# kimkyeonghun/MSA

Hardware: AMD Instinct MI355X
Metric: train-step samples/sec (higher is better)
Workload: dtype bf16

## Files before the change

msa_amd/csrc/rowwise.hip:

```cpp
#include "common.h"
#include <cstring>

std::atomic<int> g_mmb_deterministic{0};

__global__ void split_rows_kernel(const int64_t* __restrict__ row_seq, const int64_t* __restrict__ row_pos, const int* __restrict__ start_a,
                                  const int* __restrict__ start_b, const int* __restrict__ valid, int mode, int M, int rows_a,
                                  int64_t* __restrict__ perm, int64_t* __restrict__ inv, const int* __restrict__ rank,
                                  int* __restrict__ perm32, int* __restrict__ inv32) {
    const int i = blockIdx.x * blockDim.x + threadIdx.x;
    if (i >= M) return;
    const int s = (int)row_seq[i], p = rank ? rank[i] : (int)row_pos[i], v = valid[s];
    int n = rows_a;
    bool own = false;
    if (p < v) { n = start_a[s] + p; own = true; }
    else if (mode == 0) { n = start_b[s] + p - v; own = true; }
    else if (mode == 1) { n = start_b[s]; own = p == v; }
    inv[i] = n;
    if (inv32) inv32[i] = n;
    if (own) { perm[n] = i; if (perm32) perm32[n] = i; }
}

#define SL_MAXSEQ 1024
__global__ __launch_bounds__(1024) void split_layout_kernel(const int* __restrict__ lens, const int* __restrict__ valid, int nseq, int rows, int xs,
                                                            int nf_max, int nq_max, int* __restrict__ out) {
// ... 452 lines not shown
        if (r.dyr >= 0) {
            const bf16_t* dyr = dy + (size_t)r.dyr * lddy + lane * 4;
#pragma unroll
            for (int c = 0; c < NV; ++c) ndl[c] = *(const u32x2_t*)(dyr + c * 256);
        } else {
#pragma unroll
            for (int c = 0; c < NV; ++c) ndl[c] = (u32x2_t){0u, 0u};
        }
    };
    int i = blockIdx.x * WPB + w;
    if (i < M) {
        Row r0 = row_of(i);
        request(r0);
        Row r1 = row_of(i + stride);
        for (; i < M; i += stride) {
            u32x2_t dl[NV], tl[NV];
#pragma unroll
            for (int c = 0; c < NV; ++c) { dl[c] = ndl[c]; tl[c] = ntl[c]; }
            const Row r = r0;
            r0 = r1;
            if (i + stride < M) request(r0);
            r1 = row_of(i + 2 * stride);
            const uint32_t row_w = r.dr * (uint32_t)((H / 2) * MMB_WEYL);
            const float nmr = -r.mean * r.rstd;
            f32x2 g[NV][2], xh[NV][2], s1 = {0.f, 0.f}, s2 = {0.f, 0.f};
#pragma unroll
            for (int c = 0; c < NV; ++c)
#pragma unroll
                for (int k = 0; k < 2; ++k) {
                    uint32_t dw = dl[c][k];
                    if (POST) dw &= ~mmb_drop_mask2(mmb_pair_mix(row_w + lane_post + (uint32_t)(c * 128 + k) * MMB_WEYL), post_pk);
                    f32x2 dv = bf2_unpack(dw);
                    if (POST) dv *= post_scale;
                    xh[c][k] = fma2(bf2_unpack(tl[c][k]), (f32x2){r.rstd, r.rstd}, (f32x2){nmr, nmr});
                    ag[c][k] = fma2(dv, xh[c][k], ag[c][k]);
                    ab[c][k] += dv;
                    g[c][k] = dv * gam[c][k];
                    s1 += g[c][k];
                    s2 = fma2(g[c][k], xh[c][k], s2);
                }
            const float m1 = wave_sum_dpp(s1.x + s1.y) * (1.0f / H), m2 = wave_sum_dpp(s2.x + s2.y) * (1.0f / H);
            const float c1 = -m1 * r.rstd, c2 = -m2 * r.rstd;
            bf16_t* dxr = dx + (size_t)r.dxr * lddx + lane * 4;
            bf16_t* dx2r = DX2 ? dx2 + (size_t)i * lddx2 + lane * 4 : nullptr;
#pragma unroll
            for (int c = 0; c < NV; ++c) {
                u32x2_t ow, ow2;
#pragma unroll
                for (int k = 0; k < 2; ++k) {
                    const f32x2 o = fma2(xh[c][k], (f32x2){c2, c2}, fma2(g[c][k], (f32x2){r.rstd, r.rstd}, (f32x2){c1, c1}));
                    ow[k] = bf2_pack(o);
                    if (DX2 && PRE) {
                        const f32x2 o2 = o * pre_scale;
                        const uint32_t dm = mmb_drop_mask2(mmb_pair_mix(row_w + lane_pre + (uint32_t)(c * 128 + k) * MMB_WEYL), pre_pk);
                        ow2[k] = bf2_pack(o2) & ~dm;
                        const float klo = (dm & 0x8000u) ? 0.f : o2[0], khi = (dm & 0x80000000u) ? 0.f : o2[1];
                        ad[c][k] += (f32x2){klo, khi};
                    } else {
                        if (DX2) ow2[k] = ow[k];
                        if (want_ad) ad[c][k] += o;
                    }
                }
                *(u32x2_t*)(dxr + c * 256) = ow;
                if (DX2) *(u32x2_t*)(dx2r + c * 256) = ow2;
            }
        }
    }
    auto fold = [&](f32x2 (&acc)[NV][2], int slot, float* out) {
#pragma unroll
        for (int c = 0; c < NV; ++c)
#pragma unroll
            for (int k = 0; k < 2; ++k) *(f32x2*)&red[w][c * 256 + lane * 4 + 2 * k] = acc[c][k];
        __syncthreads();
        for (int col = threadIdx.x; col < H; col += WPB * 64) {
            float t = 0.f;
#pragma unroll
            for (int q = 0; q < WPB; ++q) t += red[q][col];
            if (partial) partial[((size_t)blockIdx.x * 3 + slot) * H + col] = t;
            else if (out) atomicAdd(out + col, t);
        }
        __syncthreads();
    };
    fold(ag, 0, dgamma);
    fold(ab, 1, dbeta);
    if (dbias2) fold(ad, 2, dbias2);
}


struct LnReduceBatch { float* out[32][3]; const float* partial[32]; int nblocks[32]; int H, nq, items, ordered; };
__global__ __launch_bounds__(1024) void ln_bwd_reduce_batch_kernel(const LnReduceBatch b) {
    __shared__ float red[16][64];
    const int col = blockIdx.x * 64 + (threadIdx.x & 63), sub = threadIdx.x >> 6, nsub = (int)blockDim.x >> 6;
    const int item = blockIdx.y / b.nq, k = blockIdx.y - item * b.nq;
    float* out = b.out[item][k];
    if (out == nullptr) return;
    if (b.ordered) {
        for (int j = 0; j < item; ++j)
            if (b.out[j][k] == out) return;
        float total = 0.f;
        for (int it = item; it < b.items; ++it) {
            if (b.out[it][k] != out) continue;
            const float* partial = b.partial[it];
            const int nblocks = b.nblocks[it];
            float s = 0.f;
            if (col < b.H)
                for (int q = sub; q < nblocks; q += nsub) s += partial[((size_t)q * b.nq + k) * b.H + col];
            red[sub][threadIdx.x & 63] = s;
            __syncthreads();
            if (sub == 0) {
                float t = red[0][threadIdx.x];
                for (int q = 1; q < nsub; ++q) t += red[q][threadIdx.x];
                total += t;
            }
            __syncthreads();
        }
        if (sub == 0 && col < b.H) out[col] += total;
        return;
    }
    const float* partial = b.partial[item];
    const int nblocks = b.nblocks[item];
    const int per = (nblocks + gridDim.z - 1) / gridDim.z;
    const int b0 = blockIdx.z * per, b1 = min(nblocks, b0 + per);
    float s = 0.f;
    if (col < b.H)
        for (int q = b0 + sub; q < b1; q += nsub) s += partial[((size_t)q * b.nq + k) * b.H + col];
    red[sub][threadIdx.x & 63] = s;
    __syncthreads();
    if (sub == 0 && col < b.H) {
        float t = red[0][threadIdx.x];
        for (int q = 1; q < nsub; ++q) t += red[q][threadIdx.x];
        atomicAdd(out + col, t);
    }
}

__global__ __launch_bounds__(256) void embed_gather_kernel(const int64_t* __restrict__ ids, const int64_t* __restrict__ tts,
                                                           const float* __restrict__ word, const float* __restrict__ type,
                                                           const float* __restrict__ pos, int n, int T, int H, int V,
                                                           bf16_t* __restrict__ out, int ldo) {
    const int lane = threadIdx.x & 63;
    for (int i = blockIdx.x * 4 + (threadIdx.x >> 6); i < n; i += gridDim.x * 4) {
        long id = ids[i]; if (id < 0 || id >= V) id = 0;
        const long tt = tts ? (tts[i] != 0) : 0;
        const float* wr = word + (size_t)id * H;
        const float* tr = type + (size_t)tt * H;
        const float* pr = pos + (size_t)(i % T) * H;
        for (int col = lane * 4; col < H; col += 256) {
            const float4 a = *(const float4*)(wr + col), b = *(const float4*)(tr + col), c = *(const float4*)(pr + col);
            bf16x4 o = {f2bf(a.x + b.x + c.x), f2bf(a.y + b.y + c.y), f2bf(a.z + b.z + c.z), f2bf(a.w + b.w + c.w)};
            *(bf16x4*)(out + (size_t)i * ldo + col) = o;
        }
    }
}

__global__ __launch_bounds__(256) void embed_scatter_kernel(const int64_t* __restrict__ ids, const int64_t* __restrict__ tts,
                                                            const bf16_t* __restrict__ d, int ldd, int n, int T, int H, int V,
                                                            float* __restrict__ gword, float* __restrict__ gtype, float* __restrict__ gpos,
                                                            float* __restrict__ type_slab) {
    const int p = blockIdx.x;
    for (int col = threadIdx.x * 4; col < H; col += 1024) {
        float ps[4] = {0.f, 0.f, 0.f, 0.f}, t0[4] = {0.f, 0.f, 0.f, 0.f}, t1[4] = {0.f, 0.f, 0.f, 0.f};
        for (int i0 = p + (int)blockIdx.y * 8 * T; i0 < n; i0 += 8 * T * (int)gridDim.y) {
            long id[8]; bool tt[8]; bf16x4 v[8];
#pragma unroll
            for (int u = 0; u < 8; ++u) {
                const int i = min(i0 + u * T, n - 1);
                id[u] = ids[i];
                tt[u] = tts ? (tts[i] != 0) : false;
                v[u] = *(const bf16x4*)(d + (size_t)i * ldd + col);
            }
#pragma unroll
            for (int u = 0; u < 8; ++u) {
                if (i0 + u * T >= n) break;
                const bool word = gword != nullptr && id[u] > 0 && id[u] < V;
#pragma unroll
                for (int r = 0; r < 4; ++r) {
                    const float f = bf2f(v[u][r]);
                    ps[r] += f;
                    if (tt[u]) t1[r] += f; else t0[r] += f;
                    if (word) atomicAdd(gword + (size_t)id[u] * H + col + r, f);
                }
            }
        }
#pragma unroll
        for (int r = 0; r < 4; ++r) {
            atomicAdd(gpos + (size_t)p * H + col + r, ps[r]);
            if (type_slab) { type_slab[((size_t)p * 2) * H + col + r] = t0[r]; type_slab[((size_t)p * 2 + 1) * H + col + r] = t1[r]; }
            else {
                if (t0[r] != 0.f) atomicAdd(gtype + col + r, t0[r]);
                if (t1[r] != 0.f) atomicAdd(gtype + H + col + r, t1[r]);
            }
        }
    }
}

template <int KSHIFT, typename FT>
__global__ __launch_bounds__(256) void pair_proj_fwd_kernel(const FT* __restrict__ feat, int n_rows, int P, int D,
                                                            const float* __restrict__ W, const float* __restrict__ bias, int H,
                                                            bf16_t* __restrict__ out, int ldo, int T, int KC, int pitch) {
#if defined(__gfx950__)
    extern __shared__ __attribute__((aligned(16))) float pair_sm[];
    float* Ws = pair_sm;
    float* Fs = pair_sm + 128 * pitch;
    const int tid = threadIdx.x, wave = tid >> 6, lane = tid & 63, c = lane & 15, g = lane >> 4;
    const int row0 = blockIdx.x * 64, h0 = blockIdx.y * 128;
    const int wh = (wave & 1) * 64, wr = (wave >> 1) * 32;
    f32x4 acc[4][2];
#pragma unroll
    for (int i = 0; i < 4; ++i)
#pragma unroll
        for (int j = 0; j < 2; ++j) acc[i][j] = (f32x4){0.f, 0.f, 0.f, 0.f};
    float bcol[4][4];
#pragma unroll
    for (int i = 0; i < 4; ++i)
#pragma unroll
        for (int q = 0; q < 4; ++q) bcol[i][q] = bias[min(h0 + wh + 16 * i + 4 * g + q, H - 1)];
    constexpr int kw = 1 << KSHIFT, rstep = 256 >> KSHIFT;
    const int kl = tid & (kw - 1), rsub = tid >> KSHIFT;
    for (int k0 = 0; k0 < D; k0 += KC) {
        const int kc = min(KC, D - k0), kc4 = (kc + 3) & ~3;
        if (k0) __syncthreads();
        const float kmask = kl < kc ? 1.f : 0.f;
        const int kg = min(k0 + kl, D - 1);
        const bool kst = kl < kc4;
        auto stage = [&](auto base, int g0, int lim, int lrow0, auto nrows_c) {
            constexpr int N = decltype(nrows_c)::value / rstep, NB = N < 32 ? N : 32;
#pragma unroll 1
            for (int ub = 0; ub < N; ub += NB) {
                std::remove_cv_t<std::remove_reference_t<decltype(base[0])>> v[NB];
#pragma unroll
                for (int u = 0; u < NB; ++u) {
                    const int gr = g0 + rsub + (ub + u) * rstep;
                    v[u] = base[(uint32_t)(min(gr, lim - 1) * D + kg)];
                }
                if (kst) {
#pragma unroll
                    for (int u = 0; u < NB; ++u) {
                        const int r = rsub + (ub + u) * rstep;
                        pair_sm[(lrow0 + r) * pitch + kl] = (float)v[u] * (g0 + r < lim ? kmask : 0.f);
                    }
                }
            }
        };
        stage(W, h0, H, 0, std::integral_constant<int, 128>{});
        stage(feat, row0, n_rows, 128, std::integral_constant<int, 64>{});
        __syncthreads();
        const float* wa = Ws + (wh + c) * pitch + g;
        const float* fb = Fs + (wr + c) * pitch + g;
        float av[4], bv[2];
#pragma unroll
        for (int i = 0; i < 4; ++i) av[i] = wa[16 * i * pitch];
#pragma unroll
        for (int j = 0; j < 2; ++j) bv[j] = fb[16 * j * pitch];
        for (int kk = 0; kk < kc4; kk += 4) {
            float an[4], bn[2];
            const int kn = kk + 4 < kc4 ? kk + 4 : kk;
#pragma unroll
            for (int i = 0; i < 4; ++i) an[i] = wa[16 * i * pitch + kn];
#pragma unroll
            for (int j = 0; j < 2; ++j) bn[j] = fb[16 * j * pitch + kn];
            __builtin_amdgcn_sched_barrier(0);
#pragma unroll
            for (int i = 0; i < 4; ++i)
#pragma unroll
                for (int j = 0; j < 2; ++j) acc[i][j] = __builtin_amdgcn_mfma_f32_16x16x4f32(av[i], bv[j], acc[i][j], 0, 0, 0);
            __builtin_amdgcn_sched_barrier(0);
#pragma unroll
            for (int i = 0; i < 4; ++i) av[i] = an[i];
#pragma unroll
            for (int j = 0; j < 2; ++j) bv[j] = bn[j];
        }
    }
    if (h0 + 128 <= H && !(ldo & 7)) {
        __syncthreads();
        bf16_t* Os = (bf16_t*)pair_sm;
#pragma unroll
        for (int j = 0; j < 2; ++j)
#pragma unroll
            for (int i = 0; i < 4; ++i) {
                bf16x4 ov = {f2bf(fmaxf(acc[i][j][0] + bcol[i][0], 0.f)), f2bf(fmaxf(acc[i][j][1] + bcol[i][1], 0.f)),
                             f2bf(fmaxf(acc[i][j][2] + bcol[i][2], 0.f)), f2bf(fmaxf(acc[i][j][3] + bcol[i][3], 0.f))};
                *(bf16x4*)(Os + (wr + 16 * j + c) * 136 + wh + 16 * i + 4 * g) = ov;
            }
        __syncthreads();
#pragma unroll
        for (int ps = 0; ps < 4; ++ps) {
            const int rl = (tid >> 4) + 16 * ps, row = row0 + rl;
            if (row >= n_rows) continue;
            const int b_ = row / P, p_ = row - b_ * P;
            *(bf16x8*)(out + (size_t)(b_ * (T + P) + T + p_) * ldo + h0 + 8 * (tid & 15)) = *(const bf16x8*)(Os + rl * 136 + 8 * (tid & 15));
        }
        return;
    }
#pragma unroll
    for (int j = 0; j < 2; ++j) {
        const int row = row0 + wr + 16 * j + c;
        if (row >= n_rows) continue;
        const int b_ = row / P, p_ = row - b_ * P;
        bf16_t* orow = out + (size_t)(b_ * (T + P) + T + p_) * ldo;
#pragma unroll
        for (int i = 0; i < 4; ++i) {
            const int h = h0 + wh + 16 * i + 4 * g;
            if (h + 3 < H && !(ldo & 3)) {
                bf16x4 ov = {f2bf(fmaxf(acc[i][j][0] + bcol[i][0], 0.f)), f2bf(fmaxf(acc[i][j][1] + bcol[i][1], 0.f)),
                             f2bf(fmaxf(acc[i][j][2] + bcol[i][2], 0.f)), f2bf(fmaxf(acc[i][j][3] + bcol[i][3], 0.f))};
                *(bf16x4*)(orow + h) = ov;
            } else {
#pragma unroll
                for (int q = 0; q < 4; ++q) if (h + q < H) orow[h + q] = f2bf(fmaxf(acc[i][j][q] + bcol[i][q], 0.f));
            }
        }
    }
#endif
}

struct PairBwdArgs { const void* feat; const bf16_t* J; const bf16_t* dJ; float* slab; int n, P, D, T, H, ld, rows_per_wg, ntiles; };
constexpr int PAIR_NT = 5;

template <typename FT>
__global__ __launch_bounds__(256) void pair_wgrad_kernel(const PairBwdArgs a) {
#if defined(__gfx950__)
    __shared__ float red[3][PAIR_NT * 16][64];
    const int tid = threadIdx.x, wave = tid >> 6, lane = tid & 63, c = lane & 15, g = lane >> 4;
    const int hb = blockIdx.x * 64, s = blockIdx.y, jt0 = blockIdx.z * PAIR_NT;
    const int njt = min(PAIR_NT, a.ntiles - jt0);
    const int rpw = a.rows_per_wg >> 2;
    const int r0 = s * a.rows_per_wg + wave * rpw, r1 = min(r0 + rpw, a.n);
    const int hcol = hb + 4 * c;
    const bool hok = hcol + 3 < a.H;
    struct Stage { bf16x4 j, d; float f[PAIR_NT]; };
    auto load = [&](Stage& st, int r) {
        const bool ok = r < r1;
        const int rc = ok ? r : 0;
        const int b_ = rc / a.P, p_ = rc - b_ * a.P;
        const size_t off = (size_t)(b_ * (a.T + a.P) + a.T + p_) * a.ld + (hok ? hcol : 0);
        st.j = *(const bf16x4*)(a.J + off);
        st.d = *(const bf16x4*)(a.dJ + off);
        const FT* fr = (const FT*)a.feat + (size_t)rc * a.D;
#pragma unroll
        for (int j = 0; j < PAIR_NT; ++j) {
            const int k = (jt0 + j) * 16 + c;
            const float live = (ok && j < njt) ? 1.0f : 0.0f;
            st.f[j] = fmaf((float)fr[min(k, a.D - 1)], k < a.D ? live : 0.0f, k == a.D ? live : 0.0f);
        }
// ... 12 lines not shown
#pragma unroll
        for (int u = 0; u < 4; ++u) {
            float av[4];
#pragma unroll
            for (int i = 0; i < 4; ++i) av[i] = bf2f(st[u].j[i]) > 0.f ? bf2f(st[u].d[i]) : 0.f;
            float fv[PAIR_NT];
#pragma unroll
            for (int j = 0; j < PAIR_NT; ++j) fv[j] = st[u].f[j];
            load(st[u], r + 16 + 4 * u + g);
#pragma unroll
            for (int j = 0; j < PAIR_NT; ++j) {
                if (j >= njt) continue;
#pragma unroll
                for (int i = 0; i < 4; ++i) acc[j][i] = __builtin_amdgcn_mfma_f32_16x16x4f32(av[i], fv[j], acc[j][i], 0, 0, 0);
            }
        }
    }
    if (wave) {
#pragma unroll
        for (int j = 0; j < PAIR_NT; ++j)
#pragma unroll
            for (int i = 0; i < 4; ++i)
#pragma unroll
                for (int q = 0; q < 4; ++q) red[wave - 1][(j * 4 + i) * 4 + q][lane] = acc[j][i][q];
    }
    __syncthreads();
    if (wave == 0) {
        const int W1 = a.D + 1;
        float* out = a.slab + (size_t)s * a.H * W1;
#pragma unroll
        for (int j = 0; j < PAIR_NT; ++j) {
            const int k = (jt0 + j) * 16 + c;
#pragma unroll
            for (int i = 0; i < 4; ++i)
#pragma unroll
                for (int q = 0; q < 4; ++q) {
                    const int e = (j * 4 + i) * 4 + q;
                    const float v = ((acc[j][i][q] + red[0][e][lane]) + red[1][e][lane]) + red[2][e][lane];
                    const int h = hb + 4 * (4 * g + q) + i;
                    if (j < njt && k < W1 && h < a.H) out[(size_t)h * W1 + k] = v;
                }
        }
    }
#endif
}

__global__ void pair_wgrad_reduce_kernel(const float* __restrict__ slab, int S, int H, int D, float* __restrict__ dW, float* __restrict__ db) {
    const int i = blockIdx.x * blockDim.x + threadIdx.x;
    const int W1 = D + 1;
    if (i >= H * W1) return;
    float t = 0.f;
    int s_ = 0;
    for (; s_ + 8 <= S; s_ += 8) {
        float v[8];
#pragma unroll
        for (int u = 0; u < 8; ++u) v[u] = slab[(size_t)(s_ + u) * H * W1 + i];
#pragma unroll
        for (int u = 0; u < 8; ++u) t += v[u];
    }
    for (; s_ < S; ++s_) t += slab[(size_t)s_ * H * W1 + i];
    const int h = i / W1, k = i - h * W1;
    if (k < D) dW[(size_t)h * D + k] += t; else db[h] += t;
}

__global__ __launch_bounds__(1024) void active_rows_kernel(const int64_t* __restrict__ labels, int M, int V, int* __restrict__ idx, int* __restrict__ count) {
    __shared__ int wsum[16];
    __shared__ int base;
    const int tid = threadIdx.x, lane = tid & 63, w = tid >> 6;
    if (tid == 0) base = 0;
    __syncthreads();
    for (int i0 = 0; i0 < M; i0 += 1024) {
        const int i = i0 + tid;
        const bool act = i < M && labels[i] >= 0 && labels[i] < V;
        const unsigned long long bal = __ballot(act);
        const int before = __popcll(bal & ((1ull << lane) - 1ull));
        if (lane == 0) wsum[w] = __popcll(bal);
        __syncthreads();
        int off = base;
        for (int q = 0; q < w; ++q) off += wsum[q];
        if (act) idx[off + before] = i;
        __syncthreads();
        if (tid == 0) { int t = 0; for (int q = 0; q < 16; ++q) t += wsum[q]; base += t; }
        __syncthreads();
    }
    if (tid == 0) *count = base;
}

__global__ void ce_count_kernel(const int64_t* __restrict__ labels, int M, int V, const int* __restrict__ seg_bounds, int nseg,
                                float* __restrict__ inv_count, float* __restrict__ loss_sum) {
    __shared__ int cnt[4];
    if (threadIdx.x < 4) cnt[threadIdx.x] = 0;
    __syncthreads();
    const int b1 = nseg > 1 ? seg_bounds[1] : 0x7fffffff, b2 = nseg > 2 ? seg_bounds[2] : 0x7fffffff, b3 = nseg > 3 ? seg_bounds[3] : 0x7fffffff;
    int c[4] = {0, 0, 0, 0};
    for (int i0 = threadIdx.x; i0 < M; i0 += (int)blockDim.x * 8) {
        int64_t lab[8];
#pragma unroll
        for (int u = 0; u < 8; ++u) lab[u] = labels[min(i0 + u * (int)blockDim.x, M - 1)];
#pragma unroll
        for (int u = 0; u < 8; ++u) {
            const int i = i0 + u * (int)blockDim.x;
            const int ok = (i < M && lab[u] >= 0 && lab[u] < V) ? 1 : 0;
            const int sg = (i >= b1 ? 1 : 0) + (i >= b2 ? 1 : 0) + (i >= b3 ? 1 : 0);
#pragma unroll
            for (int q = 0; q < 4; ++q) c[q] += (sg == q) ? ok : 0;
        }
    }
#pragma unroll
    for (int q = 0; q < 4; ++q) if (c[q]) atomicAdd(&cnt[q], c[q]);
    __syncthreads();
    if (threadIdx.x < nseg) {
        inv_count[threadIdx.x] = 1.0f / (float)max(cnt[threadIdx.x], 1);
        loss_sum[threadIdx.x] = 0.f;
    }
}

__global__ __launch_bounds__(1024) void ce_loss_sum_ordered_kernel(const float* __restrict__ row_loss, int M, const int* __restrict__ seg_bounds, int nseg,
                                                                   float* __restrict__ loss_sum) {
    __shared__ float red[4][1024];
    const int b1 = nseg > 1 ? seg_bounds[1] : 0x7fffffff, b2 = nseg > 2 ? seg_bounds[2] : 0x7fffffff, b3 = nseg > 3 ? seg_bounds[3] : 0x7fffffff;
    float c[4] = {0.f, 0.f, 0.f, 0.f};
    for (int i0 = threadIdx.x; i0 < M; i0 += 1024 * 8) {
        float v[8];
#pragma unroll
        for (int u = 0; u < 8; ++u) v[u] = row_loss[min(i0 + u * 1024, M - 1)];
#pragma unroll
        for (int u = 0; u < 8; ++u) {
            const int i = i0 + u * 1024;
            const int sg = (i >= b1 ? 1 : 0) + (i >= b2 ? 1 : 0) + (i >= b3 ? 1 : 0);
            const float x = i < M ? v[u] : 0.f;
#pragma unroll
            for (int q = 0; q < 4; ++q) c[q] += (sg == q) ? x : 0.f;
        }
    }
#pragma unroll
    for (int q = 0; q < 4; ++q) red[q][threadIdx.x] = c[q];
    __syncthreads();
    for (int w = 512; w > 0; w >>= 1) {
        if ((int)threadIdx.x < w) {
#pragma unroll
            for (int q = 0; q < 4; ++q) red[q][threadIdx.x] += red[q][threadIdx.x + w];
        }
        __syncthreads();
    }
    if ((int)threadIdx.x < nseg) loss_sum[threadIdx.x] = red[threadIdx.x][0];
}

#define RUNS_MAXN 8192
__global__ __launch_bounds__(1024) void id_runs_sum_rows_kernel(const void* __restrict__ src, int src_bf16, int lds, const int64_t* __restrict__ ids,
                                                                int n, int H, int V, const int64_t* __restrict__ uni, int U,
                                                                float* __restrict__ dst, int ldd) {
    __shared__ int list[RUNS_MAXN];
    __shared__ float red[1024 * 4];
    __shared__ int s_count, s_earlier;
    const int i0 = blockIdx.x, tid = threadIdx.x, nthr = blockDim.x;
    const long long key = ids[i0];
    if (key <= 0 || key >= V) return;
    if (tid == 0) { s_count = 0; s_earlier = 0; }
    __syncthreads();
    int earlier = 0;
    for (int j = tid; j < i0; j += nthr) earlier |= (ids[j] == key) ? 1 : 0;
    if (earlier) s_earlier = 1;
    __syncthreads();
    if (s_earlier) return;
    long long dr = key;
    if (uni) {
        int lo = 0, hi = U - 1;
        while (lo < hi) { const int mid = (lo + hi) >> 1; if (uni[mid] < key) lo = mid + 1; else hi = mid; }
        if (U <= 0 || uni[lo] != key) return;
        dr = lo;
    }
    if (tid < 64) {
        int count = 0;
        for (int base = i0; base < n; base += 64) {
            const int j = base + tid;
            const bool hit = j < n && ids[j] == key;
            const unsigned long long m = __ballot(hit);
            if (hit) list[count + __popcll(m & ((1ull << tid) - 1ull))] = j;
            count += __popcll(m);
        }
        if (tid == 0) s_count = count;
    }
    __syncthreads();
    const int cnt = s_count;
    const int CT = H >> 2, G = nthr / CT;
    const int g = tid / CT, c = tid - g * CT;
    float a[4] = {0.f, 0.f, 0.f, 0.f};
    if (g < G) {
#pragma unroll 4
        for (int k = g; k < cnt; k += G) {
            const size_t r = (size_t)list[k];
            if (src_bf16) {
                const bf16x4 x = *(const bf16x4*)((const bf16_t*)src + r * lds + 4 * c);
#pragma unroll
                for (int q = 0; q < 4; ++q) a[q] += bf2f(x[q]);
            } else {
                const float4 x = *(const float4*)((const float*)src + r * lds + 4 * c);
                a[0] += x.x; a[1] += x.y; a[2] += x.z; a[3] += x.w;
            }
        }
#pragma unroll
        for (int q = 0; q < 4; ++q) red[(g * CT + c) * 4 + q] = a[q];
    }
    __syncthreads();
    if (g == 0) {
        float4* d = (float4*)(dst + (size_t)dr * ldd + 4 * c);
        float4 o = *d;
        float t[4] = {0.f, 0.f, 0.f, 0.f};
        for (int gg = 0; gg < G; ++gg)
#pragma unroll
            for (int q = 0; q < 4; ++q) t[q] += red[(gg * CT + c) * 4 + q];
        o.x += t[0]; o.y += t[1]; o.z += t[2]; o.w += t[3];
        *d = o;
    }
}

__global__ void embed_type_fold_kernel(const float* __restrict__ slab, int T, int H, float* __restrict__ gtype) {
    const int e = blockIdx.x * blockDim.x + threadIdx.x;
    if (e >= 2 * H) return;
    float t = 0.f;
    for (int p = 0; p < T; ++p) t += slab[(size_t)p * 2 * H + e];
    gtype[e] += t;
}

#define CE_MAXC 16
template <int MODE, bool F32, bool SMOOTH = false>
__global__ __launch_bounds__(256) void ce_row_kernel(const void* __restrict__ logits_, int ldv, int V, const int64_t* __restrict__ labels,
                                                     const int* __restrict__ seg_bounds, int nseg, const float* __restrict__ inv_count,
                                                     float* __restrict__ loss_sum, float* __restrict__ row_lse, const float* __restrict__ gscale,
                                                     bf16_t* __restrict__ dlogits, int ldd, const int* __restrict__ rows, float* __restrict__ row_loss,
                                                     float one_minus, float eps_over_v) {
    __shared__ float red[4];
    __shared__ float lab_logit;
    const int i = rows ? rows[blockIdx.x] : blockIdx.x;
    const int64_t lab = labels[i];
    const int tid = threadIdx.x, lane = tid & 63, w = tid >> 6;
    const int nchunk = ldv >> 3;
    if (lab < 0 || lab >= V) {
        if (MODE == 0) { if (tid == 0) { row_lse[i] = 0.f; if (row_loss) row_loss[i] = 0.f; } }
        else {
            bf16_t* drow = dlogits + (size_t)(rows ? blockIdx.x : i) * ldd;
            const bf16x8 z = {0, 0, 0, 0, 0, 0, 0, 0};
            for (int c = tid; c < nchunk; c += 256) *(bf16x8*)(drow + c * 8) = z;
        }
        return;
    }
    int s = 0;
    while (s + 1 < nseg && i >= seg_bounds[s + 1]) ++s;
    bf16x8 v[CE_MAXC];
    if constexpr (F32) {
        const float* row = (const float*)logits_ + (size_t)i * ldv;
#pragma unroll
        for (int c = 0; c < CE_MAXC; ++c) {
            const int ch = c * 256 + tid;
            if (ch < nchunk) {
                const float4 lo = *(const float4*)(row + ch * 8), hi = *(const float4*)(row + ch * 8 + 4);
                v[c] = (bf16x8){f2bf(lo.x), f2bf(lo.y), f2bf(lo.z), f2bf(lo.w), f2bf(hi.x), f2bf(hi.y), f2bf(hi.z), f2bf(hi.w)};
            }
        }
    } else {
        const bf16_t* row = (const bf16_t*)logits_ + (size_t)i * ldv;
#pragma unroll
        for (int c = 0; c < CE_MAXC; ++c) {
            const int ch = c * 256 + tid;
            if (ch < nchunk) v[c] = *(const bf16x8*)(row + ch * 8);
        }
    }
    if (MODE == 0) {
        float mx = -INFINITY;
#pragma unroll
        for (int c = 0; c < CE_MAXC; ++c) {
            const int ch = c * 256 + tid;
            if (ch < nchunk) {
#pragma unroll
                for (int r = 0; r < 8; ++r) if (ch * 8 + r < V) mx = fmaxf(mx, bf2f(v[c][r]));
            }
        }
        mx = wave_max(mx);
        if (lane == 0) red[w] = mx;
        __syncthreads();
        mx = fmaxf(fmaxf(red[0], red[1]), fmaxf(red[2], red[3]));
        __syncthreads();
        float se = 0.f;
        float sx = 0.f;
#pragma unroll
        for (int c = 0; c < CE_MAXC; ++c) {
            const int ch = c * 256 + tid;
            if (ch < nchunk) {
#pragma unroll
                for (int r = 0; r < 8; ++r) if (ch * 8 + r < V) {
                    se += __expf(bf2f(v[c][r]) - mx);
                    if constexpr (SMOOTH) sx += bf2f(v[c][r]);
                }
                if ((int)(lab >> 3) == ch) lab_logit = bf2f(v[c][lab & 7]);
            }
        }
        se = wave_sum(se);
        if (lane == 0) red[w] = se;
        if constexpr (SMOOTH) {
            __shared__ float red_x[4];
            sx = wave_sum(sx);
            if (lane == 0) red_x[w] = sx;
            __syncthreads();
            if (tid == 0) {
                const float lse = mx + __logf(red[0] + red[1] + red[2] + red[3]);
                const float sum_x = ((red_x[0] + red_x[1]) + red_x[2]) + red_x[3];
                row_lse[i] = lse;
                const float term = __fmaf_rn(-eps_over_v, sum_x, __fmaf_rn(-one_minus, lab_logit, lse)) * inv_count[s];
                if (row_loss) row_loss[i] = term;
                else atomicAdd(loss_sum + s, term);
            }
            return;
        }
        __syncthreads();
        if (tid == 0) {
            const float lse = mx + __logf(red[0] + red[1] + red[2] + red[3]);
            row_lse[i] = lse;
            if (row_loss) row_loss[i] = (lse - lab_logit) * inv_count[s];
            else atomicAdd(loss_sum + s, (lse - lab_logit) * inv_count[s]);
        }
    } else {
        const float lse = row_lse[i];
        const float scale = inv_count[s] * gscale[s];
        bf16_t* drow = dlogits + (size_t)(rows ? blockIdx.x : i) * ldd;
#pragma unroll
        for (int c = 0; c < CE_MAXC; ++c) {
            const int ch = c * 256 + tid;
            if (ch < nchunk) {
                bf16x8 o;
#pragma unroll
                for (int r = 0; r < 8; ++r) {
                    const int col = ch * 8 + r;
                    float pr = col < V ? __expf(bf2f(v[c][r]) - lse) : 0.f;
                    if constexpr (SMOOTH) {
                        if (col == (int)lab) pr -= one_minus;
                        if (col < V) pr -= eps_over_v;
                    } else {
                        if (col == (int)lab) pr -= 1.0f;
                    }
                    o[r] = f2bf(pr * scale);
                }
                *(bf16x8*)(drow + ch * 8) = o;
            }
        }
    }
}

typedef uint32_t vt_u32x4 __attribute__((ext_vector_type(4)));

__device__ __forceinline__ uint32_t vt_key(uint32_t h) {
    const uint32_t neg = (uint32_t)((int32_t)h >> 31);
    return h ^ ((neg & 0x7FFF0000u) | 0x80000000u);
}
__device__ __forceinline__ float vt_value(uint32_t word) {
    const uint32_t kk = word & 0xFFFF0000u;
    return __builtin_bit_cast(float, (kk & 0x80000000u) ? (kk ^ 0x80000000u) : (kk ^ 0xFFFF0000u));
}
__device__ __forceinline__ uint32_t vt_wave_max(uint32_t v) {
#pragma unroll
    for (int o = 32; o > 0; o >>= 1) v = max(v, (uint32_t)__shfl_xor((int)v, o, 64));
    return v;
}
template <bool COUNT>
__device__ __forceinline__ uint32_t vt_scan(const uint32_t (&e)[CE_MAXC * 8], uint32_t prev, uint32_t lab_word, int& above) {
    uint32_t best = 0u;
#pragma unroll
    for (int n = 0; n < CE_MAXC * 8; ++n) {
        best = max(best, e[n] - prev);
        if (COUNT) above += e[n] > lab_word ? 1 : 0;
    }
    const uint32_t word = best + prev;
    return word < prev ? word : 0u;
}

// ... 745 lines not shown
        if (int e = mmb_allow_lds((const void*)pair_proj_fwd_kernel<7, FT>, 192 * 130 * (int)sizeof(float), attr_done)) return e;
        hipLaunchKernelGGL((pair_proj_fwd_kernel<7, FT>), dim3((n + 63) / 64, (H + 127) / 128), dim3(256), lds, stream, feat, n, P, D, W, bias, H, (bf16_t*)out, ldo, T,
                           KC, pitch);
    }
    MMB_CHECK_LAUNCH();
    return 0;
}

extern "C" {

uint32_t mmbert_rng_stream(uint64_t seed, uint32_t site) {
    uint32_t a = mmb_hash32((uint32_t)seed ^ 0xA511E9B3u);
    uint32_t b = mmb_hash32((uint32_t)(seed >> 32) + 0x7F4A7C15u);
    return mmb_hash32(a ^ (b * 0x9E3779B1u) ^ mmb_hash32(site * 0x85EBCA6Bu + 0x27D4EB2Fu));
}

uint32_t mmbert_dropout_thr16(float p) {
    if (p <= 0.f) return 0;
    double t = (double)p * 65536.0 + 0.5;
    if (t > 65535.0) t = 65535.0;
    return (uint32_t)t;
}

static inline bool ln_lean(int H) { return (H & 255) == 0 && H <= LN_MAXV * 256; }

int mmbert_ln_fwd(hipStream_t stream, const void* x, int ldx, const int* in_rows, void* y, int ldy, const int* out_rows,
                  int M, int H, const float* gamma, const float* beta, float eps, float* mean, float* rstd,
                  uint32_t dstream, uint32_t dthr, float dscale, int drop_row0) {
    if (M <= 0) return 0;
    if (H > LN_MAXV * 256 || (H & 3) || (ldx & 3) || (ldy & 3)) return -1;
    constexpr int cap = 0;
    if (ln_lean(H)) {
        const int NVL = H >> 8;
        const dim3 grid(grid_for(M, 4, cap > 0 ? cap : 1024));
#define LN_FWD_LEAN(NVV, DD) hipLaunchKernelGGL((ln_fwd_lean_kernel<NVV, DD>), grid, dim3(256), 0, stream, (const bf16_t*)x, ldx, in_rows, \
                                                 (bf16_t*)y, ldy, out_rows, M, gamma, beta, eps, mean, rstd, dstream, dthr, dscale, drop_row0)
        if (dthr) { if (NVL == 1) LN_FWD_LEAN(1, true); else if (NVL == 2) LN_FWD_LEAN(2, true); else if (NVL == 3) LN_FWD_LEAN(3, true); else LN_FWD_LEAN(4, true); }
        else { if (NVL == 1) LN_FWD_LEAN(1, false); else if (NVL == 2) LN_FWD_LEAN(2, false); else if (NVL == 3) LN_FWD_LEAN(3, false); else LN_FWD_LEAN(4, false); }
#undef LN_FWD_LEAN
        MMB_CHECK_LAUNCH();
        return 0;
    }
    const int R = M >= 8192 ? 2 : 1;
    const int NV = (H + 255) / 256;
#define LN_FWD_LAUNCH(NVV, RR) hipLaunchKernelGGL((ln_fwd_kernel<NVV, RR>), dim3(grid_for(M, 4 * RR, cap > 0 ? cap : 2048)), dim3(256), 0, stream, (const bf16_t*)x, ldx, in_rows, \
                                                  (bf16_t*)y, ldy, out_rows, M, H, gamma, beta, eps, mean, rstd, dstream, dthr, dscale, drop_row0)
    if (R >= 2) { if (NV == 1) LN_FWD_LAUNCH(1, 2); else if (NV == 2) LN_FWD_LAUNCH(2, 2); else if (NV == 3) LN_FWD_LAUNCH(3, 2); else LN_FWD_LAUNCH(4, 2); }
    else { if (NV == 1) LN_FWD_LAUNCH(1, 1); else if (NV == 2) LN_FWD_LAUNCH(2, 1); else if (NV == 3) LN_FWD_LAUNCH(3, 1); else LN_FWD_LAUNCH(4, 1); }
#undef LN_FWD_LAUNCH
    MMB_CHECK_LAUNCH();
    return 0;
}

constexpr int LN_BWD_LEAN_WPB = 8;
static inline int ln_bwd_lean_wpb() { return LN_BWD_LEAN_WPB; }
static inline int ln_bwd_blocks(int M, int H) {
    constexpr int cap_env = 0;
    if (ln_lean(H)) {
        const int wpb = ln_bwd_lean_wpb();
        return grid_for(M, wpb, cap_env > 0 ? cap_env : (wpb == 8 ? 256 : 512));
    }
    return grid_for(M, 4, cap_env > 0 ? cap_env : 1024);
}

int mmbert_ln_bwd(hipStream_t stream, const void* dy, int lddy, const int* dy_rows, const void* x, int ldx, const int* x_rows,
                  const float* mean, const float* rstd, const float* gamma, int M, int H,
                  void* dx, int lddx, const int* dx_rows, void* dx2, int lddx2, float* dgamma, float* dbeta, float* dbias2,
                  uint32_t post_stream, uint32_t post_thr, float post_scale,
                  uint32_t pre_stream, uint32_t pre_thr, float pre_scale, float* partial_ws, const int* drop_rows, int defer_reduce,
                  int dy_row_limit) {
    if (M <= 0) return 0;
    if (H > LN_MAXV * 256 || (H & 3) || (ldx & 3) || (lddy & 3) || (lddx & 3) || (lddx2 & 3)) return -1;
    if (dy_row_limit > 0 && !dy_rows) return -1;
    if (defer_reduce && !partial_ws) return -1;
    const int nblocks = ln_bwd_blocks(M, H);
    if (ln_lean(H)) {
        const int NVL = H >> 8;
        const bool post = post_thr != 0, has2 = dx2 != nullptr, pre = has2 && pre_thr != 0;
        const int wpb = ln_bwd_lean_wpb();
#define LN_BWD_LEAN(NVV, PO, D2, PR, WW) hipLaunchKernelGGL((ln_bwd_lean_kernel<NVV, PO, D2, PR, WW>), dim3(nblocks), dim3(WW * 64), 0, stream, (const bf16_t*)dy, lddy, dy_rows, \
        (const bf16_t*)x, ldx, x_rows, mean, rstd, gamma, M, (bf16_t*)dx, lddx, dx_rows, (bf16_t*)dx2, lddx2, dgamma, dbeta, dbias2, partial_ws, \
        post_stream, post_thr, post_scale, pre_stream, pre_thr, pre_scale, drop_rows, dy_row_limit)
#define LN_BWD_LEAN_W(NVV, WW) { if (post) { if (!has2) LN_BWD_LEAN(NVV, true, false, false, WW); else if (pre) LN_BWD_LEAN(NVV, true, true, true, WW); else LN_BWD_LEAN(NVV, true, true, false, WW); } \
                                 else { if (!has2) LN_BWD_LEAN(NVV, false, false, false, WW); else if (pre) LN_BWD_LEAN(NVV, false, true, true, WW); else LN_BWD_LEAN(NVV, false, true, false, WW); } }
#define LN_BWD_LEAN_NV(NVV) { if (wpb == 8) LN_BWD_LEAN_W(NVV, 8) else LN_BWD_LEAN_W(NVV, 4) }
        if (NVL == 1) LN_BWD_LEAN_NV(1) else if (NVL == 2) LN_BWD_LEAN_NV(2) else if (NVL == 3) LN_BWD_LEAN_NV(3) else LN_BWD_LEAN_NV(4)
#undef LN_BWD_LEAN_NV
#undef LN_BWD_LEAN_W
#undef LN_BWD_LEAN
    } else {
    const int R = 1;
    const int NV = (H + 255) / 256;
#define LN_BWD_LAUNCH(NVV, RR) hipLaunchKernelGGL((ln_bwd_kernel<NVV, RR>), dim3(nblocks), dim3(256), 0, stream, (const bf16_t*)dy, lddy, dy_rows, \
        (const bf16_t*)x, ldx, x_rows, mean, rstd, gamma, M, H, (bf16_t*)dx, lddx, dx_rows, (bf16_t*)dx2, lddx2, dgamma, dbeta, dbias2, partial_ws, \
        post_stream, post_thr, post_scale, pre_stream, pre_thr, pre_scale, drop_rows, dy_row_limit)
    if (R >= 2) { if (NV == 1) LN_BWD_LAUNCH(1, 2); else if (NV == 2) LN_BWD_LAUNCH(2, 2); else if (NV == 3) LN_BWD_LAUNCH(3, 2); else LN_BWD_LAUNCH(4, 2); }
    else { if (NV == 1) LN_BWD_LAUNCH(1, 1); else if (NV == 2) LN_BWD_LAUNCH(2, 1); else if (NV == 3) LN_BWD_LAUNCH(3, 1); else LN_BWD_LAUNCH(4, 1); }
#undef LN_BWD_LAUNCH
    }
    MMB_CHECK_LAUNCH();
    if (partial_ws && !defer_reduce) {
        LnReduceBatch b = {};
        b.out[0][0] = dgamma; b.out[0][1] = dbeta; b.out[0][2] = dbias2; b.partial[0] = partial_ws;
        b.nblocks[0] = nblocks; b.H = H; b.nq = 3; b.items = 1; b.ordered = mmb_deterministic() ? 1 : 0;
        hipLaunchKernelGGL(ln_bwd_reduce_batch_kernel, dim3((H + 63) / 64, 3, b.ordered ? 1 : 8), dim3(b.ordered ? 1024 : 256), 0, stream, b);
        MMB_CHECK_LAUNCH();
    }
    return 0;
}

size_t mmbert_ln_bwd_workspace(int M, int H) { return (size_t)ln_bwd_blocks(M, H) * 3 * H; }

static int ln_bwd_reduce_launch(hipStream_t stream, int items, const float* const* partial_ws, float* const* dgamma, float* const* dbeta,
                                float* const* dbias2, const int* Ms, int M_all, int H) {
    if (items <= 0) return 0;
    if (items > 32) return -1;
    LnReduceBatch b = {};
    for (int i = 0; i < items; ++i) {
        const int M = Ms ? Ms[i] : M_all;
        b.out[i][0] = M > 0 ? dgamma[i] : nullptr; b.out[i][1] = M > 0 ? dbeta[i] : nullptr; b.out[i][2] = (M > 0 && dbias2) ? dbias2[i] : nullptr;
        b.partial[i] = partial_ws[i];
        b.nblocks[i] = M > 0 ? ln_bwd_blocks(M, H) : 0;
    }
    b.H = H; b.nq = 3; b.items = items; b.ordered = mmb_deterministic() ? 1 : 0;
    hipLaunchKernelGGL(ln_bwd_reduce_batch_kernel, dim3((H + 63) / 64, items * 3, b.ordered ? 1 : 8), dim3(b.ordered ? 1024 : 256), 0, stream, b);
    MMB_CHECK_LAUNCH();
    return 0;
}
int mmbert_ln_bwd_reduce(hipStream_t stream, int items, const float* const* partial_ws, float* const* dgamma, float* const* dbeta,
                         float* const* dbias2, int M, int H) {
    if (M <= 0) return 0;
    return ln_bwd_reduce_launch(stream, items, partial_ws, dgamma, dbeta, dbias2, nullptr, M, H);
}
int mmbert_ln_bwd_reduce_rows(hipStream_t stream, int items, const float* const* partial_ws, float* const* dgamma, float* const* dbeta,
                              float* const* dbias2, const int* M, int H) {
    if (!M) return -1;
    return ln_bwd_reduce_launch(stream, items, partial_ws, dgamma, dbeta, dbias2, M, 0, H);
}

int mmbert_embed_gather(hipStream_t stream, const int64_t* ids, const int64_t* tts, const float* word, const float* type, const float* pos,
                        int n, int T, int H, int V, void* out, int ldo) {
    if (n <= 0) return 0;
    if ((H & 3) || (ldo & 3)) return -1;
    hipLaunchKernelGGL(embed_gather_kernel, dim3(grid_for(n, 4)), dim3(256), 0, stream, ids, tts, word, type, pos, n, T, H, V, (bf16_t*)out, ldo);
    MMB_CHECK_LAUNCH();
    return 0;
}

int mmbert_embed_scatter(hipStream_t stream, const int64_t* ids, const int64_t* tts, const void* d, int ldd, int n, int T, int H, int V,
                         float* gword, float* gtype, float* gpos, float* type_slab) {
    if (n <= 0) return 0;
    if (H > LN_MAXV * 256 || (H & 3) || (ldd & 3) || T <= 0) return -1;
    if (mmb_deterministic() && (gword != nullptr || type_slab == nullptr)) return -4;
    constexpr int slices = 1;
    hipLaunchKernelGGL(embed_scatter_kernel, dim3(T < n ? T : n, slices), dim3(256), 0, stream, ids, tts, (const bf16_t*)d, ldd, n, T, H, V, gword, gtype, gpos, type_slab);
    MMB_CHECK_LAUNCH();
    if (type_slab) {
        hipLaunchKernelGGL(embed_type_fold_kernel, dim3((2 * H + 255) / 256), dim3(256), 0, stream, type_slab, T < n ? T : n, H, gtype);
        MMB_CHECK_LAUNCH();
    }
    return 0;
}

int mmbert_pair_proj_fwd(hipStream_t stream, const void* feat, int feat_f64, int B, int P, int D, const float* W, const float* bias, int H,
                         void* out, int ldo, int T) {
    const int n = B * P;
    if (n <= 0) return 0;
    if (D < 1 || H < 1) return -1;
    const int KC = D < 128 ? (D + 3) & ~3 : 128;
    const int pitch = KC + ((18 - (KC & 15)) & 15);
    const int ops_lds = 192 * pitch * (int)sizeof(float), out_lds = 64 * 136 * (int)sizeof(bf16_t);
    const int lds = ops_lds > out_lds ? ops_lds : out_lds;
    return feat_f64 ? pair_proj_fwd_launch(stream, (const double*)feat, n, P, D, W, bias, H, out, ldo, T, KC, pitch, lds)
                    : pair_proj_fwd_launch(stream, (const float*)feat, n, P, D, W, bias, H, out, ldo, T, KC, pitch, lds);
}

static void pair_bwd_split(int n, int D, int H, int* rows_per_wg, int* S) {
    const int htiles = (H + 63) / 64, zt = ((D + 1 + 15) / 16 + PAIR_NT - 1) / PAIR_NT;
    int want = (mmb_device_cus() + htiles * zt - 1) / (htiles * zt);
    if (want < 1) want = 1;
    int rp = ((n + want - 1) / want + 63) / 64 * 64;
    if (rp < 64) rp = 64;
    *rows_per_wg = rp;
    *S = (n + rp - 1) / rp;
}
size_t mmbert_pair_proj_bwd_workspace(int B, int P, int D, int H) {
    if (B <= 0 || P <= 0 || D < 1 || H < 1) return 0;
    int rp, S;
    pair_bwd_split(B * P, D, H, &rp, &S);
    return (size_t)S * H * (D + 1) * sizeof(float);
}

int mmbert_pair_proj_bwd(hipStream_t stream, const void* feat, int feat_f64, int B, int P, int D, const void* J, const void* dJ, int ld, int T,
                         float* dW, float* db, int H, void* workspace) {
    const int n = B * P;
    if (n <= 0) return 0;
    if (!workspace || (H & 7) || (ld & 7) || D < 1) return -1;
    PairBwdArgs a = {};
    a.feat = feat; a.J = (const bf16_t*)J; a.dJ = (const bf16_t*)dJ; a.slab = (float*)workspace;
    a.n = n; a.P = P; a.D = D; a.T = T; a.H = H; a.ld = ld;
    int S;
    pair_bwd_split(n, D, H, &a.rows_per_wg, &S);
    a.ntiles = (D + 1 + 15) / 16;
    const dim3 grid((H + 63) / 64, S, (a.ntiles + PAIR_NT - 1) / PAIR_NT);
    if (feat_f64) hipLaunchKernelGGL(pair_wgrad_kernel<double>, grid, dim3(256), 0, stream, a);
    else hipLaunchKernelGGL(pair_wgrad_kernel<float>, grid, dim3(256), 0, stream, a);
    MMB_CHECK_LAUNCH();
    hipLaunchKernelGGL(pair_wgrad_reduce_kernel, dim3((H * (D + 1) + 255) / 256), dim3(256), 0, stream, (const float*)workspace, S, H, D, dW, db);
    MMB_CHECK_LAUNCH();
    return 0;
}

static bool ce_smoothing_ok(float smoothing) { return smoothing >= 0.f && smoothing < 1.f; }

static int ce_fwd_launch(hipStream_t stream, const void* logits, int ldv, int V, const int64_t* labels, int M, const int* seg_bounds, int nseg,
                         float* inv_count, float* loss_sum, float* row_lse, int logits_f32, float* row_loss, float smoothing) {
    if (M <= 0) return 0;
    if (nseg < 1 || nseg > 4 || (ldv & 7) || ldv > CE_MAXC * 256 * 8 || V > ldv) return -1;
    if (smoothing != 0.f && V < 1) return -1;
    const bool det = mmb_deterministic();
    if (det && !row_loss) return -4;
    if (!det) row_loss = nullptr;
    hipLaunchKernelGGL(ce_count_kernel, dim3(1), dim3(1024), 0, stream, labels, M, V, seg_bounds, nseg, inv_count, loss_sum);
    MMB_CHECK_LAUNCH();
    if (smoothing != 0.f) {
        const float one_minus = 1.f - smoothing, eps_over_v = smoothing / (float)V;
        if (logits_f32)
            hipLaunchKernelGGL((ce_row_kernel<0, true, true>), dim3(M), dim3(256), 0, stream, logits, ldv, V, labels, seg_bounds, nseg, inv_count,
                               loss_sum, row_lse, (const float*)nullptr, (bf16_t*)nullptr, 0, (const int*)nullptr, row_loss, one_minus, eps_over_v);
        else
            hipLaunchKernelGGL((ce_row_kernel<0, false, true>), dim3(M), dim3(256), 0, stream, logits, ldv, V, labels, seg_bounds, nseg, inv_count,
                               loss_sum, row_lse, (const float*)nullptr, (bf16_t*)nullptr, 0, (const int*)nullptr, row_loss, one_minus, eps_over_v);
    } else if (logits_f32)
        hipLaunchKernelGGL((ce_row_kernel<0, true>), dim3(M), dim3(256), 0, stream, logits, ldv, V, labels, seg_bounds, nseg, inv_count, loss_sum,
                           row_lse, (const float*)nullptr, (bf16_t*)nullptr, 0, (const int*)nullptr, row_loss, 1.f, 0.f);
    else
        hipLaunchKernelGGL((ce_row_kernel<0, false>), dim3(M), dim3(256), 0, stream, logits, ldv, V, labels, seg_bounds, nseg, inv_count, loss_sum,
                           row_lse, (const float*)nullptr, (bf16_t*)nullptr, 0, (const int*)nullptr, row_loss, 1.f, 0.f);
    MMB_CHECK_LAUNCH();
    if (det) {
        hipLaunchKernelGGL(ce_loss_sum_ordered_kernel, dim3(1), dim3(1024), 0, stream, (const float*)row_loss, M, seg_bounds, nseg, loss_sum);
        MMB_CHECK_LAUNCH();
    }
    return 0;
}

int mmbert_ce_fwd(hipStream_t stream, const void* logits, int ldv, int V, const int64_t* labels, int M,
                  const int* seg_bounds, int nseg, float* inv_count, float* loss_sum, float* row_lse, int logits_f32, float* row_loss) {
    return ce_fwd_launch(stream, logits, ldv, V, labels, M, seg_bounds, nseg, inv_count, loss_sum, row_lse, logits_f32, row_loss, 0.f);
}

int mmbert_ce_fwd_smooth(hipStream_t stream, const void* logits, int ldv, int V, const int64_t* labels, int M, const int* seg_bounds, int nseg,
                         float* inv_count, float* loss_sum, float* row_lse, int logits_f32, float* row_loss, float smoothing) {
    if (!ce_smoothing_ok(smoothing)) return -1;
    return ce_fwd_launch(stream, logits, ldv, V, labels, M, seg_bounds, nseg, inv_count, loss_sum, row_lse, logits_f32, row_loss, smoothing);
}

int mmbert_vocab_topk(hipStream_t stream, const void* logits, int ldv, int V, int M, int logits_f32, int k, const int64_t* labels,
                      int32_t* top_ids, float* top_logprob, float* row_lse, float* label_logprob, int32_t* label_rank) {
    if (M < 0 || V < 1 || V > CE_MAXC * 256 * 8 || k < 1 || k > 8 || k > V || (ldv & 7) || ldv < V) return -1;
    if (M == 0) return 0;
    if (!logits || !top_ids || !top_logprob || !row_lse) return -1;
    if (labels ? (!label_logprob || !label_rank) : (label_logprob || label_rank)) return -1;
    if (logits_f32)
        hipLaunchKernelGGL(vocab_topk_kernel<true>, dim3(M), dim3(256), 0, stream, logits, ldv, V, k, labels, top_ids, top_logprob, row_lse,
                           label_logprob, label_rank);
    else
        hipLaunchKernelGGL(vocab_topk_kernel<false>, dim3(M), dim3(256), 0, stream, logits, ldv, V, k, labels, top_ids, top_logprob, row_lse,
                           label_logprob, label_rank);
    MMB_CHECK_LAUNCH();
    return 0;
}

void mmbert_set_deterministic(int on) { g_mmb_deterministic.store(on != 0); }
int mmbert_get_deterministic(void) { return g_mmb_deterministic.load(); }

int mmbert_id_runs_sum_rows(hipStream_t stream, const void* src, int src_bf16, int lds, const int64_t* ids, int n,
                            int H, int V, const int64_t* uni, int U, float* dst, int ldd) {
    if (n <= 0) return 0;
    if ((H & 3) || H > 4096 || n > RUNS_MAXN || (lds & 3) || (ldd & 3) || !src || !ids || !dst) return -1;
    const int CT = H >> 2;
    int G = 1024 / CT; if (G > 8) G = 8; if (G < 1) G = 1;
    int threads = G * CT; if (threads < 64) threads = 64;
    hipLaunchKernelGGL(id_runs_sum_rows_kernel, dim3(n), dim3(threads), 0, stream, src, src_bf16, lds, ids, n, H, V, uni, U, dst, ldd);
    MMB_CHECK_LAUNCH();
    return 0;
}

static int ce_bwd_launch(hipStream_t stream, const void* logits, int ldv, int V, const int64_t* labels, int M, const int* seg_bounds, int nseg,
                         const float* inv_count, const float* gscale, const float* row_lse, void* dlogits, int ldd, const int* rows, int nrows,
                         int logits_f32, float smoothing) {
    if (M <= 0 || (rows && nrows <= 0)) return 0;
    if (nseg < 1 || nseg > 4 || (ldv & 7) || (ldd & 7) || ldv > CE_MAXC * 256 * 8 || V > ldv) return -1;
    if (smoothing != 0.f && V < 1) return -1;
    if (smoothing != 0.f) {
        const float one_minus = 1.f - smoothing, eps_over_v = smoothing / (float)V;
        if (logits_f32)
            hipLaunchKernelGGL((ce_row_kernel<1, true, true>), dim3(rows ? nrows : M), dim3(256), 0, stream, logits, ldv, V, labels, seg_bounds, nseg,
                               inv_count, (float*)nullptr, (float*)row_lse, gscale, (bf16_t*)dlogits, ldd, rows, (float*)nullptr, one_minus, eps_over_v);
        else
            hipLaunchKernelGGL((ce_row_kernel<1, false, true>), dim3(rows ? nrows : M), dim3(256), 0, stream, logits, ldv, V, labels, seg_bounds, nseg,
                               inv_count, (float*)nullptr, (float*)row_lse, gscale, (bf16_t*)dlogits, ldd, rows, (float*)nullptr, one_minus, eps_over_v);
    } else if (logits_f32)
        hipLaunchKernelGGL((ce_row_kernel<1, true>), dim3(rows ? nrows : M), dim3(256), 0, stream, logits, ldv, V, labels, seg_bounds, nseg, inv_count,
                           (float*)nullptr, (float*)row_lse, gscale, (bf16_t*)dlogits, ldd, rows, (float*)nullptr, 1.f, 0.f);
    else
        hipLaunchKernelGGL((ce_row_kernel<1, false>), dim3(rows ? nrows : M), dim3(256), 0, stream, logits, ldv, V, labels, seg_bounds, nseg, inv_count,
                           (float*)nullptr, (float*)row_lse, gscale, (bf16_t*)dlogits, ldd, rows, (float*)nullptr, 1.f, 0.f);
// ... 376 lines not shown
```

Baseline: 1261.

## Restructure embedding scatter, id-run list build, and type-fold reduction for parallelism

```diff
diff --git a/msa_amd/csrc/rowwise.hip b/msa_amd/csrc/rowwise.hip
--- a/msa_amd/csrc/rowwise.hip
+++ b/msa_amd/csrc/rowwise.hip
@@ -628,43 +628,50 @@
     }
 }
 
-__global__ __launch_bounds__(256) void embed_scatter_kernel(const int64_t* __restrict__ ids, const int64_t* __restrict__ tts,
-                                                            const bf16_t* __restrict__ d, int ldd, int n, int T, int H, int V,
-                                                            float* __restrict__ gword, float* __restrict__ gtype, float* __restrict__ gpos,
-                                                            float* __restrict__ type_slab) {
-    const int p = blockIdx.x;
-    for (int col = threadIdx.x * 4; col < H; col += 1024) {
-        float ps[4] = {0.f, 0.f, 0.f, 0.f}, t0[4] = {0.f, 0.f, 0.f, 0.f}, t1[4] = {0.f, 0.f, 0.f, 0.f};
-        for (int i0 = p + (int)blockIdx.y * 8 * T; i0 < n; i0 += 8 * T * (int)gridDim.y) {
-            long id[8]; bool tt[8]; bf16x4 v[8];
-#pragma unroll
-            for (int u = 0; u < 8; ++u) {
-                const int i = min(i0 + u * T, n - 1);
-                id[u] = ids[i];
-                tt[u] = tts ? (tts[i] != 0) : false;
-                v[u] = *(const bf16x4*)(d + (size_t)i * ldd + col);
-            }
-#pragma unroll
-            for (int u = 0; u < 8; ++u) {
-                if (i0 + u * T >= n) break;
-                const bool word = gword != nullptr && id[u] > 0 && id[u] < V;
-#pragma unroll
-                for (int r = 0; r < 4; ++r) {
-                    const float f = bf2f(v[u][r]);
-                    ps[r] += f;
-                    if (tt[u]) t1[r] += f; else t0[r] += f;
-                    if (word) atomicAdd(gword + (size_t)id[u] * H + col + r, f);
-                }
-            }
-        }
-#pragma unroll
-        for (int r = 0; r < 4; ++r) {
-            atomicAdd(gpos + (size_t)p * H + col + r, ps[r]);
-            if (type_slab) { type_slab[((size_t)p * 2) * H + col + r] = t0[r]; type_slab[((size_t)p * 2 + 1) * H + col + r] = t1[r]; }
-            else {
-                if (t0[r] != 0.f) atomicAdd(gtype + col + r, t0[r]);
-                if (t1[r] != 0.f) atomicAdd(gtype + H + col + r, t1[r]);
-            }
+#define ES_ROWS 48
+__global__ __launch_bounds__(64) void embed_scatter_kernel(const int64_t* __restrict__ ids, const int64_t* __restrict__ tts,
+                                                           const bf16_t* __restrict__ d, int ldd, int n, int T, int H, int V,
+                                                           float* __restrict__ gword, float* __restrict__ gtype, float* __restrict__ gpos,
+                                                           float* __restrict__ type_slab) {
+#pragma clang fp reassociate(off)
+    const int p = blockIdx.x, lane = threadIdx.x;
+    const int col = ((int)blockIdx.y * 64 + lane) * 4;
+    const bool live = col < H;
+    const int lcol = live ? col : 0;
+    float ps[4] = {0.f, 0.f, 0.f, 0.f}, t0[4] = {0.f, 0.f, 0.f, 0.f}, t1[4] = {0.f, 0.f, 0.f, 0.f};
+    for (int i0 = p; i0 < n; i0 += ES_ROWS * T) {
+        const int iu = min(i0 + lane * T, n - 1);
+        const long idl = gword ? ids[iu] : 0;
+        const int widl = (idl > 0 && idl < V) ? (int)idl : 0;
+        const unsigned long long tt = __ballot(tts ? tts[iu] != 0 : false);
+        bf16x4 v[ES_ROWS];
+#pragma unroll
+        for (int u = 0; u < ES_ROWS; ++u) {
+            const int i = min(i0 + u * T, n - 1);
+            v[u] = *(const bf16x4*)(d + (size_t)i * ldd + lcol);
+        }
+#pragma unroll
+        for (int u = 0; u < ES_ROWS; ++u) {
+            if (i0 + u * T >= n) break;
+            const bool t = (tt >> u) & 1ull;
+            const int wid = __builtin_amdgcn_readlane(widl, u);
+#pragma unroll
+            for (int r = 0; r < 4; ++r) {
+                const float f = bf2f(v[u][r]);
+                ps[r] += f;
+                if (t) t1[r] += f; else t0[r] += f;
+                if (wid && live) atomicAdd(gword + (size_t)wid * H + col + r, f);
+            }
+        }
+    }
+    if (!live) return;
+#pragma unroll
+    for (int r = 0; r < 4; ++r) {
+        atomicAdd(gpos + (size_t)p * H + col + r, ps[r]);
+        if (type_slab) { type_slab[((size_t)p * 2) * H + col + r] = t0[r]; type_slab[((size_t)p * 2 + 1) * H + col + r] = t1[r]; }
+        else {
+            if (t0[r] != 0.f) atomicAdd(gtype + col + r, t0[r]);
+            if (t1[r] != 0.f) atomicAdd(gtype + H + col + r, t1[r]);
         }
     }
 }
@@ -983,11 +990,11 @@
                                                                 float* __restrict__ dst, int ldd) {
     __shared__ int list[RUNS_MAXN];
     __shared__ float red[1024 * 4];
-    __shared__ int s_count, s_earlier;
+    __shared__ int s_wcount[16], s_earlier;
     const int i0 = blockIdx.x, tid = threadIdx.x, nthr = blockDim.x;
     const long long key = ids[i0];
     if (key <= 0 || key >= V) return;
-    if (tid == 0) { s_count = 0; s_earlier = 0; }
+    if (tid == 0) s_earlier = 0;
     __syncthreads();
     int earlier = 0;
     for (int j = tid; j < i0; j += nthr) earlier |= (ids[j] == key) ? 1 : 0;
@@ -1001,19 +1008,19 @@
         if (U <= 0 || uni[lo] != key) return;
         dr = lo;
     }
-    if (tid < 64) {
-        int count = 0;
-        for (int base = i0; base < n; base += 64) {
-            const int j = base + tid;
-            const bool hit = j < n && ids[j] == key;
-            const unsigned long long m = __ballot(hit);
-            if (hit) list[count + __popcll(m & ((1ull << tid) - 1ull))] = j;
-            count += __popcll(m);
-        }
-        if (tid == 0) s_count = count;
-    }
-    __syncthreads();
-    const int cnt = s_count;
+    const int lane = tid & 63, w = tid >> 6, nw = (nthr + 63) >> 6;
+    int cnt = 0;
+    for (int j0 = i0; j0 < n; j0 += nthr) {
+        const int j = j0 + tid;
+        const bool hit = j < n && ids[j] == key;
+        const unsigned long long m = __ballot(hit);
+        if (lane == 0) s_wcount[w] = __popcll(m);
+        __syncthreads();
+        int off = cnt;
+        for (int q = 0; q < nw; ++q) { const int c = s_wcount[q]; if (q < w) off += c; cnt += c; }
+        if (hit) list[off + __popcll(m & ((1ull << lane) - 1ull))] = j;
+        __syncthreads();
+    }
     const int CT = H >> 2, G = nthr / CT;
     const int g = tid / CT, c = tid - g * CT;
     float a[4] = {0.f, 0.f, 0.f, 0.f};
@@ -1047,10 +1054,20 @@
 }
 
 __global__ void embed_type_fold_kernel(const float* __restrict__ slab, int T, int H, float* __restrict__ gtype) {
+#pragma clang fp reassociate(off)
     const int e = blockIdx.x * blockDim.x + threadIdx.x;
     if (e >= 2 * H) return;
-    float t = 0.f;
-    for (int p = 0; p < T; ++p) t += slab[(size_t)p * 2 * H + e];
+    const int T2 = T & ~1;
+    float te = 0.f, to = 0.f;
+    for (int p0 = 0; p0 < T2; p0 += 16) {
+        float v[16];
+#pragma unroll
+        for (int u = 0; u < 16; ++u) v[u] = slab[(size_t)min(p0 + u, T - 1) * 2 * H + e];
+#pragma unroll
+        for (int u = 0; u < 16; u += 2) if (p0 + u < T2) { te += v[u]; to += v[u + 1]; }
+    }
+    float t = te + to;
+    if (T & 1) t += slab[(size_t)(T - 1) * 2 * H + e];
     gtype[e] += t;
 }
 
@@ -2102,8 +2119,8 @@
     if (n <= 0) return 0;
     if (H > LN_MAXV * 256 || (H & 3) || (ldd & 3) || T <= 0) return -1;
     if (mmb_deterministic() && (gword != nullptr || type_slab == nullptr)) return -4;
-    constexpr int slices = 1;
-    hipLaunchKernelGGL(embed_scatter_kernel, dim3(T < n ? T : n, slices), dim3(256), 0, stream, ids, tts, (const bf16_t*)d, ldd, n, T, H, V, gword, gtype, gpos, type_slab);
+    hipLaunchKernelGGL(embed_scatter_kernel, dim3(T < n ? T : n, (H + 255) / 256), dim3(64), 0, stream, ids, tts, (const bf16_t*)d, ldd, n, T, H, V, gword, gtype,
+                       gpos, type_slab);
     MMB_CHECK_LAUNCH();
     if (type_slab) {
         hipLaunchKernelGGL(embed_type_fold_kernel, dim3((2 * H + 255) / 256), dim3(256), 0, stream, type_slab, T < n ? T : n, H, gtype);
```

Result: no change. 1251 (-0.8%).
